# Gustavroot/DeflatedMLMC_Schwinger

Measured on AMD Instinct MI355X. Metric: hutchinson_probe_samples_per_sec_schwinger128, higher is better.
Workload: dtype f64

## Files before the change

### deflatedmlmc_schwinger_amd/csrc/sw_engine.hip

```cpp
#include "../../include/schwinger_hip.h"
#include "sw_kernels.hpp"
#include "sw_pack.hpp"
#include "sw_poly.hpp"

#include <dlfcn.h>

#include <algorithm>
#include <chrono>
#include <cmath>
#include <complex>
#include <cstdarg>
#include <cstdio>
#include <cstdlib>
#include <cstring>
#include <functional>
#include <map>
#include <mutex>
#include <string>
#include <type_traits>
#include <vector>

using swk::cplx;
using swk::cplxf;
using swk::PtrList;
// ... 66 lines not shown
  cplx* h2 = nullptr;
  cplx* c1 = nullptr;
  cplx* nrm = nullptr;
  cplx* gram = nullptr;
};

struct Level {
  int n = 0;
  bool stencil = false;
  int L = 0;
  double mass = 0.0;
  cplx* U1 = nullptr;
  cplx* U2 = nullptr;
  EllOp A, P, R;
  EllOp Re;
  EllOp dinv;
  int nu_pre = 0, nu_post = 3, kcycle = 0;
  std::vector<std::complex<double>> w_pre, w_post;
  bool rich = false;
  std::vector<std::complex<double>> w_eo;
  std::vector<std::complex<double>> q_w;
  std::complex<double> q_beta;
  EllOp eo_op[5];
  std::vector<int> h_rowmap;
  int* rowmap = nullptr;
  int ws_nbp = 0;
  cplx *b = nullptr, *x = nullptr, *r = nullptr, *t = nullptr;
  cplxf *U1f = nullptr, *U2f = nullptr;
  int ws32_nbp = 0;
  cplxf *b32 = nullptr, *x32 = nullptr, *r32 = nullptr, *t32 = nullptr, *i32 = nullptr, *o32 = nullptr;
  int gm_m = 0, gm_cycles = 0;
  cplx *g1 = nullptr, *g2 = nullptr;
  KrylovWS gws;
  cplx *tv = nullptr, *tv2 = nullptr;
  KrylovWS kws;
  KrylovWS sws;
};

struct Hier {
  int nlevels = 0;
  Level lv[SW_MAX_LEVELS];
  EllOp cinv;
  bool ready = false;
  bool f32_valid = false;
  bool even_valid = false;
};
// ... 33 lines not shown
  int mfma_small_tiles = 2;
  int sync_hint[SW_MAX_HIER][SW_MAX_LEVELS] = {{0}};
  bool lazy_sync = true;
  int eo_skew = -1;
  bool eo_skew_chunk = false;
  bool gram_cycle = true;
  bool eo_product = true;
  int gj_block = 32;
  int eo_tile = 0;
  int dense_lds = 4;
  int eo_tile_dbg = 0;
  int num_cus = 256;
  bool direct_small = true;
  bool lgmres_aug = true;
  bool stencil_nt = false;
  int stencil_tile = 0;
  int stencil_spw = 0;
  bool cgs2 = false;
  bool verify = true;
  bool inner_cgs2 = false;
  bool pyth_last = true;
  bool eo_solve = true;
  bool eo_direct = true;
  bool precond_f32 = false;
  int kd = 0;
  cplx* U = nullptr;
  int defl_gemm = 0;
  int lkd[SW_MAX_LEVELS] = {0};
  cplx* lV[SW_MAX_LEVELS] = {nullptr};
  int* perm_src[SW_MAX_LEVELS] = {nullptr};
  EllOp rhsmap[SW_MAX_LEVELS];
  cplx* partial = nullptr;
  size_t partial_bytes = 0;
  cplx* small = nullptr;
  size_t small_bytes = 0;
  void* stage = nullptr;
  size_t stage_bytes = 0;
  std::vector<std::pair<void*, size_t>> allocs;
  int pb_level = -1, pb_nb = 0, pb_nbp = 0;
  int8_t* pb_probes = nullptr;
  struct ProbeSlot {
    int8_t* p = nullptr;
    size_t bytes = 0;
    int level = -1, nb = 0;
    hipEvent_t ready = nullptr;
    bool pending = false;
// ... 100 lines not shown
                                "gj_block must be 0 or a multiple of 8 in 8..256"),
    field<&sw_engine::stencil_nt>("stencil_nt"),
    field<&sw_engine::stencil_tile>("stencil_tile"),
    field<&sw_engine::stencil_spw>("stencil_spw",
                                   [](double v) {
                                     const int t = (int)v;
                                     return t == 0 || t == 1 || t == 2 || t == 4 || t == 8;
                                   },
                                   "stencil_spw must be 0,1,2,4,8"),
    field<&sw_engine::eo_tile>("eo_tile", [](double v) { return v == 0.0 || v == 4.0 || v == 8.0; },
                               "eo_tile must be 0 (off), 4 or 8 waves"),
    {"eo_tile_dbg", get_field<&sw_engine::eo_tile_dbg>, [](sw_engine* h, double v) { h->eo_tile_dbg = (int)v & 3; }},
    field<&sw_engine::eo_skew>("eo_skew", [](double v) { return !(v < -1.0 || v > 65536.0); },
                               "eo_skew must be -1 (automatic), 0 (off) or a strip height"),
    field<&sw_engine::eo_skew_chunk>("eo_skew_chunk"),
    field<&sw_engine::eo_product>("eo_product"),
    field<&sw_engine::p_even>("p_even"),
    {"ell_order", get_field<&sw_engine::ell_order>, [](sw_engine* h, double v) {
       h->ell_order = v != 0.0;
       for (Hier& H : h->hier) H.even_valid = false;
     }},
    field<&sw_engine::direct_small>("direct_small"),
    field<&sw_engine::eo_direct>("eo_direct"),
    field<&sw_engine::lgmres_aug>("lgmres_aug"),
    field<&sw_engine::cgs2>("cgs2"),
    field<&sw_engine::inner_cgs2>("inner_cgs2"),
    field<&sw_engine::pyth_last>("pyth_last"),
    field<&sw_engine::verify>("verify"),
    field<&sw_engine::lazy_sync>("lazy_sync"),
    field<&sw_engine::eo_solve>("eo_solve"),
    field<&sw_engine::gram_cycle>("gram_cycle"),
    field<&sw_engine::stop_factor>("stop_factor", [](double v) { return v > 0.0 && v <= 1.0; },
                                   "stop_factor must be in (0, 1]"),
    field<&sw_engine::precond_f32>("precond_f32"),
    field<&sw_engine::f32_krylov>("f32_krylov"),
    field<&sw_engine::f32_pairs>("f32_pairs"),
    field<&sw_engine::f32_tiles>("f32_tiles",
                                 [](double v) { const int t = (int)v; return t == 0 || t == 1 || t == 2 || t == 4; },
                                 "f32_tiles must be 0, 1, 2 or 4"),
    field<&sw_engine::f32_stages>("f32_stages"),
    field<&sw_engine::f32_dense_stages>("f32_dense_stages"),
    field<&sw_engine::f32_splitk>("f32_splitk"),
    field<&sw_engine::bench_what>("bench_what", [](double v) { return !(v < 0.0 || v > 3.0); },
                                  "bench_what must be 0..3"),
    field<&sw_engine::bench_mode>("bench_mode", [](double v) { return v == 0.0 || v == 1.0 || v == 2.0; },
                                  "bench_mode must be 0, 1 or 2"),
// ... 287 lines not shown
  for (int rt = 0; rt < RT; ++rt) {
    const int ot = tmap ? tmap[rt] : rt;
    for (int r = 0; r < 4; ++r)
      if (kcol[(size_t)rt * KS + KS - 4 + r] != 16 * ot + 4 * r) return;
  }
  op.bsr_diag_last = true;
}

static int free_op(sw_engine* h, EllOp& op) {
  SWCHK(dev_free(h, op.cols));
  SWCHK(dev_free(h, op.vals));
  SWCHK(dev_free(h, op.order));
  SWCHK(dev_free(h, op.order_even));
  SWCHK(dev_free(h, op.bsr_kcol));
  SWCHK(dev_free(h, op.bsr_vals));
  SWCHK(dev_free(h, op.bsr_tmap));
  SWCHK(dev_free(h, op.vals32));
  SWCHK(dev_free(h, op.bsr_vals32));
  op = EllOp();
  return 0;
}

static int launch_bsr(sw_engine* h, const EllOp& op, int mode, const cplx* X, const cplx* B, cplx* Y,
                      int nbp, int cat, cplx w) {
  const int RT = op.bsr_RT > 0 ? op.bsr_RT : op.nrows / 16;
  int NT = h->mfma_tiles;
  if (h->mfma_small_tiles > 0 && (long long)RT * ((2 * nbp) / (16 * NT)) < 4096)
    NT = h->mfma_small_tiles;
  const int bmap = (cat == T_COARSEST) ? h->dense_map : h->bsr_map, msub = h->bsr_sub;
  const int RBn = (RT + SW_WAVES_PER_BLOCK - 1) / SW_WAVES_PER_BLOCK, NCn = (2 * nbp) / (16 * NT);
  const int want = (cat == T_COARSEST) ? h->dense_stages : h->bsr_stages;
  const int stages = (want >= 8 && op.bsr_KS % 8 == 0) ? 8 : ((want >= 4 && op.bsr_KS % 4 == 0) ? 4 : 2);
  dim3 grid = (bmap == 0) ? dim3(RBn, NCn) : dim3(RBn * NCn);
  const int n1 = h->hier[h->solver_hid].nlevels > 1 ? h->hier[h->solver_hid].lv[1].n : 0;
  const int cls = cat == T_COARSEST ? T_MFMA_DENSE
                                    : (cat == T_MVM ? (op.nrows == n1 || n1 == 0 ? T_MFMA_OP : T_MFMA_OP2)
                                                    : cat);
  if (h->profiling) h->twork[cls] += 512.0 * (double)RT * (double)op.bsr_KS * (double)nbp;
  const int dl_kb = 4;
  if (h->mfma_3m && h->dense_lds > 0 && cat == T_COARSEST && mode == 0 && op.dense_uniform &&
      RT % h->dense_lds == 0 && op.bsr_KS % (dl_kb * SW_DL_DEPTH) == 0 && op.bsr_KS >= 2 * dl_kb * SW_DL_DEPTH &&
      (nbp & 31) == 0 && X != Y) {
    return pick<4, 2>(h->dense_lds, [&](auto RTW) {
      return launch(h, cls, swk::k_dense_mfma3_lds<RTW, dl_kb>, dim3((RT / RTW) * (nbp / 32)), dim3(128 * RTW),
                    (const cplx*)op.bsr_vals, (const int*)op.bsr_kcol, op.bsr_KS, RT, X, Y, nbp,
                    (const int*)op.bsr_tmap);
    });
  }
  if (h->mfma_3m) {
    int NT3 = 1;
    if (cat != T_COARSEST && (long long)RT * (nbp / 32) >= 16384) NT3 = 2;
    if (h->mfma3_tiles == 1 || h->mfma3_tiles == 2 || h->mfma3_tiles == 4) NT3 = h->mfma3_tiles;
    while (NT3 > 1 && nbp % (16 * NT3)) NT3 >>= 1;
    const int NC3 = nbp / (16 * NT3);
    const dim3 grid3(RBn * NC3);
    const bool ntio3 = h->bsr_nt && cat != T_COARSEST;
    const int xr = (op.bsr_diag_last && h->bsr_xreg) ? 1 : 0;
    const int bm3 = (bmap == 0) ? 0 : bmap;
    auto b3 = [&](auto MD, auto NTT, auto NTB, auto SG) {
      return launch(h, cls, swk::k_bsr_mfma3<MD, NTT, NTB, SG>, grid3, dim3(SW_BLOCK), (const cplx*)op.bsr_vals,
                    (const int*)op.bsr_kcol, op.bsr_KS, RT, X, B, Y, nbp, w, bm3, msub, (const int*)op.bsr_tmap, xr);
    };
    if (!ntio3 && mode == 0 && want >= 16 && NT3 == 1 && op.bsr_KS % 16 == 0)
      return b3(IntC<0>{}, IntC<1>{}, IntC<0>{}, IntC<16>{});
    if (!ntio3 && mode == 0 && want >= 8)
      return pick<4, 2, 1>(NT3, [&](auto NTT) { return b3(IntC<0>{}, NTT, IntC<0>{}, IntC<8>{}); });
    return pick<0, 1, 3>(mode, [&](auto MD) {
      return pick<4, 2, 1>(NT3, [&](auto NTT) {
        return pick<0, 1>(ntio3, [&](auto NTB) { return b3(MD, NTT, NTB, IntC<4>{}); });
      });
    });
  }
  const bool ntio = h->bsr_nt && cat != T_COARSEST;
  const int xr = (op.bsr_diag_last && h->bsr_xreg) ? 1 : 0;
  return pick<0, 1, 3>(mode, [&](auto MD) {
    return pick<2, 4>(NT, [&](auto NTT) {
      return pick<0, 1>(ntio, [&](auto NTB) {
        return pick<8, 4, 2>(stages, [&](auto SG) {
          return launch(h, cls, swk::k_bsr_mfma<MD, NTT, NTB, SG>, grid, dim3(SW_BLOCK), (const cplx*)op.bsr_vals,
                        (const int*)op.bsr_kcol, op.bsr_KS, RT, (const double*)X, (const double*)B, (double*)Y,
                        2 * nbp, nbp, w, bmap, msub, (const int*)op.bsr_tmap, xr);
        });
      });
    });
  });
// ... 8 lines not shown
  const dim3 grid((ng + SW_WAVES_PER_BLOCK - 1) / SW_WAVES_PER_BLOCK, nbp / 64);
  if (op.G != 1 && op.G != 2 && op.G != 4 && op.G != 8 && op.G != 16)
    return sw_fail(h, "unsupported ELL group size %d", op.G);
  return pick<1, 2, 4, 8, 16>(op.G, [&](auto G) {
    return pick<0, 1, 2, 3>(mode, [&](auto MODE) {
      return launch(h, cat, swk::k_ell<G, MODE, T>, grid, dim3(SW_BLOCK), (const int*)op.cols, vals, op.K, ng, ord,
                    X, B, Y, nbp, w);
    });
  });
}

static int launch_ell(sw_engine* h, const EllOp& op, int mode, const cplx* X, const cplx* B,
                      cplx* Y, int nbp, int cat, cplx w = cplx{0.0, 0.0}, bool even_only = false) {
  if (!op.set) return sw_fail(h, "operator not set");
  if (op.bsr_KS > 0 && (mode == 0 || mode == 1 || mode == 3) && h->use_mfma &&
      (cat == T_COARSEST || h->mfma_ops))
    return launch_bsr(h, op, mode, X, B, Y, nbp, cat, w);
  if (!op.cols || !op.vals)
    return sw_fail(h, "operator exists in MFMA block-row form only (built on the device): it needs "
                      "use_mfma = mfma_ops = 1");
  return launch_ell_groups<cplx>(h, op, op.vals, mode, X, B, Y, nbp, cat, w, even_only);
}

static int launch_bsr(sw_engine* h, const EllOp& op, int mode, const cplx* X, const cplx* B, cplx* Y,
                      int nbp, int cat, cplx w);
static int ensure_level_ws(sw_engine* h, Level& lv, int nbp);

static int apply_coarsest(sw_engine* h, Hier& H, const cplx* X, cplx* Y, int nbp) {
  Level& lc = H.lv[H.nlevels - 1];
  if (h->eo_direct && H.nlevels > 1 && lc.eo_op[4].set && lc.eo_op[1].set && lc.eo_op[2].set &&
      lc.eo_op[3].set && X != Y) {
    SWCHK(ensure_level_ws(h, lc, nbp));
    SWCHK(launch_bsr(h, lc.eo_op[1], 1, X, X, lc.r, nbp, T_MVM, cplx{0.0, 0.0}));
    SWCHK(launch_bsr(h, lc.eo_op[4], 0, lc.r, nullptr, Y, nbp, T_COARSEST, cplx{0.0, 0.0}));
    SWCHK(launch_bsr(h, lc.eo_op[2], 0, X, nullptr, Y, nbp, T_MVM, cplx{0.0, 0.0}));
    return launch_bsr(h, lc.eo_op[3], 1, Y, Y, Y, nbp, T_MVM, cplx{0.0, 0.0});
  }
  if (!H.cinv.set) return sw_fail(h, "coarsest inverse not set");
  return launch_ell(h, H.cinv, 0, X, nullptr, Y, nbp, T_COARSEST);
}

static int stencil_spw(sw_engine* h, int tile_w) {
  int spw = h->stencil_spw > 0 ? h->stencil_spw : 1;
  while (spw > 1 && tile_w % spw) spw >>= 1;
  return spw;
}

template <class C>
static swk::StencilArgsT<C> stencil_args(sw_engine* h, const Level& lv, int nbp, bool eo) {
  using S = typename swk::scalar_of<C>::type;
  swk::StencilArgsT<C> a;
  a.L = lv.L;
  a.Vh = lv.L * lv.L / 2;
  a.diag = (typename swk::real_of<C>::type)(4.0 + lv.mass);
  if constexpr (std::is_same<C, cplx>::value) {
    a.U1 = lv.U1;
    a.U2 = lv.U2;
  } else {
    a.U1 = lv.U1f;
// ... 627 lines not shown
  }
  return 0;
}

static int eo_smooth(sw_engine* h, Level& lv, const cplx* Bin, cplx* start, cplx* other, cplx* Xout,
                     int nbp) {
  cplx* bp = lv.r;
  SWCHK(eo_hop<0>(h, lv, Bin, Bin, bp, nbp));
  cplx* cur = nullptr;
  SWCHK(schur_steps(h, lv, start, other, bp, nbp, &cur));
  SWCHK(eo_hop<1>(h, lv, Bin, cur, cur, nbp));
  if (cur != Xout) return sw_fail(h, "internal: even-odd smoother ended in the wrong buffer");
  return 0;
}

static int vcycle_rich(sw_engine* h, Hier& H, int l, const cplx* Bin, cplx* Xout, int nbp) {
  Level& lv = H.lv[l];
  Level& lc = H.lv[l + 1];
  SWCHK(ensure_level_ws(h, lv, nbp));
  SWCHK(ensure_level_ws(h, lc, nbp));
  SWCHK(ensure_even_orders(h, H));
  if (!lv.P.set || !lv.R.set) return sw_fail(h, "transfer operators of level %d not set", l);
  const size_t npost = lv.w_post.size();
  if (!lv.stencil && lv.eo_op[4].set && lv.eo_op[1].set && lv.eo_op[2].set && lv.eo_op[3].set &&
      lv.w_pre.empty() && h->eo_direct) {
    SWCHK(launch_bsr(h, lv.eo_op[1], 1, Bin, Bin, lv.r, nbp, T_MVM, cplx{0.0, 0.0}));
    SWCHK(launch_bsr(h, lv.eo_op[4], 0, lv.r, nullptr, Xout, nbp, T_COARSEST, cplx{0.0, 0.0}));
    SWCHK(launch_bsr(h, lv.eo_op[2], 0, Bin, nullptr, Xout, nbp, T_MVM, cplx{0.0, 0.0}));
    return launch_bsr(h, lv.eo_op[3], 1, Xout, Xout, Xout, nbp, T_MVM, cplx{0.0, 0.0});
  }
  cplx* xpre = nullptr;
  if (!lv.w_pre.empty()) {
    SWCHK(rich_steps(h, lv, Bin, Xout, lv.t, lv.w_pre, true, nbp, &xpre));
    SWCHK(apply_op(h, lv, 1, xpre, Bin, lv.r, nbp));
    SWCHK(launch_ell(h, lv.R, 0, lv.r, nullptr, lc.b, nbp, T_R));
  } else {
    SWCHK(launch_ell(h, lv.R, 0, Bin, nullptr, lc.b, nbp, T_R));
  }
  SWCHK(coarse_correction(h, H, l, nbp));
  if (!lv.stencil && !lv.w_eo.empty() && !xpre && lv.eo_op[0].set) {
    const bool odd_steps = (lv.w_eo.size() & 1) != 0;
    cplx* cur = odd_steps ? lv.t : Xout;
    cplx* nxt = odd_steps ? Xout : lv.t;
    SWCHK(launch_ell(h, lv.P, 0, lc.x, nullptr, cur, nbp, T_P, cplx{0.0, 0.0}, true));
    SWCHK(launch_bsr(h, lv.eo_op[1], 1, Bin, Bin, lv.r, nbp, T_MVM, cplx{0.0, 0.0}));
    for (size_t k = 0; k < lv.w_eo.size(); ++k) {
      SWCHK(launch_bsr(h, lv.eo_op[0], 3, cur, lv.r, nxt, nbp, T_MVM,
                       cplx{lv.w_eo[k].real(), lv.w_eo[k].imag()}));
      std::swap(cur, nxt);
    }
    SWCHK(launch_bsr(h, lv.eo_op[2], 0, Bin, nullptr, Xout, nbp, T_MVM, cplx{0.0, 0.0}));
    return launch_bsr(h, lv.eo_op[3], 1, Xout, Xout, Xout, nbp, T_MVM, cplx{0.0, 0.0});
// ... 619 lines not shown
  if (h->h_notconv) (void)hipHostFree(h->h_notconv);
  if (h->stream) (void)hipStreamDestroy(h->stream);
  if (h->gen_stream) (void)hipStreamDestroy(h->gen_stream);
  delete h;
  return 0;
}

int sw_hier_begin(sw_engine* h, int hid, int nlevels) {
  if (!h) return 1;
  if (hid < 0 || hid >= SW_MAX_HIER) return sw_fail(h, "hierarchy id %d out of range", hid);
  if (nlevels < 1 || nlevels > SW_MAX_LEVELS) return sw_fail(h, "nlevels %d out of range", nlevels);
  HIPCHK(hipSetDevice(h->device));
  Hier& H = h->hier[hid];
  for (int l = 0; l < SW_MAX_LEVELS; ++l) h->sync_hint[hid][l] = 0;
  for (int l = 0; l < SW_MAX_LEVELS; ++l) {
    Level& lv = H.lv[l];
    SWCHK(dev_free(h, lv.U1)); SWCHK(dev_free(h, lv.U2));
    SWCHK(free_op(h, lv.A));
    SWCHK(free_op(h, lv.P));
    SWCHK(free_op(h, lv.R));
    SWCHK(free_op(h, lv.Re));
    SWCHK(free_op(h, lv.dinv));
    for (int q = 0; q < 5; ++q) SWCHK(free_op(h, lv.eo_op[q]));
    SWCHK(dev_free(h, lv.rowmap));
    SWCHK(dev_free(h, lv.b)); SWCHK(dev_free(h, lv.x)); SWCHK(dev_free(h, lv.r));
    SWCHK(dev_free(h, lv.t));
    SWCHK(dev_free(h, lv.U1f)); SWCHK(dev_free(h, lv.U2f));
    SWCHK(dev_free(h, lv.b32)); SWCHK(dev_free(h, lv.x32)); SWCHK(dev_free(h, lv.r32));
    SWCHK(dev_free(h, lv.t32)); SWCHK(dev_free(h, lv.i32)); SWCHK(dev_free(h, lv.o32));
    SWCHK(free_krylov(h, lv.kws));
    SWCHK(free_krylov(h, lv.sws));
    SWCHK(free_krylov(h, lv.gws));
    SWCHK(dev_free(h, lv.g1)); SWCHK(dev_free(h, lv.g2));
    SWCHK(dev_free(h, lv.tv)); SWCHK(dev_free(h, lv.tv2));
    lv = Level();
  }
  SWCHK(free_op(h, H.cinv));
  H.nlevels = nlevels;
  H.ready = false;
  H.f32_valid = H.even_valid = false;
  if (hid == 0) {
    h->kd = 0;
    SWCHK(dev_free(h, h->U));
    h->U = nullptr;
    for (int l = 0; l < SW_MAX_LEVELS; ++l) {
      h->lkd[l] = 0;
// ... 452 lines not shown
  SWCHK(op_to_dense(h, lv.A, n, D, nullptr));
  SWCHK(gj_invert(h, D, n));
  SWCHK(dense_to_bsr(h, H.cinv, n, D, n, nullptr, nullptr));
  return stream_sync(h);
}

int sw_get_coarsest_inv(sw_engine* h, int hid, double* dense) {
  SWCHK(check_hier(h, hid, 0, false));
  if (!dense) return sw_fail(h, "bad arguments");
  HIPCHK(hipSetDevice(h->device));
  const EllOp& op = h->hier[hid].cinv;
  if (!op.set) return sw_fail(h, "coarsest inverse missing");
  const int n = op.nrows;
  DevBuf<cplx> D(h);
  SWCHK(dev_realloc(h, &D.p, (size_t)n * n));
  SWCHK(op_to_dense(h, op, n, D, nullptr));
  HIPCHK(hipMemcpyAsync(dense, D, (size_t)n * n * sizeof(cplx), hipMemcpyDeviceToHost, h->stream));
  return stream_sync(h);
}

static int schur_apply(sw_engine* h, Level& lv, int mode, const cplx* X, const cplx* Bp, cplx* Y, int nbp);
static int dot_into(sw_engine* h, const cplx* A, const cplx* Bv, int n, int nbp, cplx* out);

int sw_setup_direct_level(sw_engine* h, int hid, int level) {
  SWCHK(check_hier(h, hid, level, false));
  HIPCHK(hipSetDevice(h->device));
  Hier& H = h->hier[hid];
  H.f32_valid = false;
  Level& lv = H.lv[level];
  const EllOp& S = lv.eo_op[0];
  if (lv.stencil || !S.set || !S.bsr_tmap || S.bsr_RT <= 0 || !lv.eo_op[1].set || !lv.eo_op[2].set ||
      !lv.eo_op[3].set)
    return sw_fail(h, "level %d has no even-odd operators (sw_setup_eo_operators / sw_set_eo_operator)", level);
  const int ne = S.bsr_RT, n = ne * 16, ns = lv.n / 16;
  if (n > 8192) return sw_fail(h, "Schur complement of %d rows too large for the in-engine dense inverse", n);
  std::vector<int> E(ne), erank(ns, -1);
  HIPCHK(hipMemcpy(E.data(), S.bsr_tmap, (size_t)ne * sizeof(int), hipMemcpyDeviceToHost));
  for (int r = 0; r < ne; ++r) {
    if (E[r] < 0 || E[r] >= ns || erank[E[r]] >= 0) return sw_fail(h, "level %d: bad tile map of the Schur operator", level);
    erank[E[r]] = r;
  }
  std::vector<int> kc((size_t)ne * S.bsr_KS);
  HIPCHK(hipMemcpy(kc.data(), S.bsr_kcol, kc.size() * sizeof(int), hipMemcpyDeviceToHost));
  for (int c : kc)
    if (erank[c >> 4] < 0) return sw_fail(h, "level %d: the Schur operator reaches an odd site", level);
  DevBuf<int> d_rank(h), d_E(h);
  SWCHK(upload(h, &d_rank.p, erank.data(), erank.size()));
  SWCHK(upload(h, &d_E.p, E.data(), E.size()));
  DevBuf<cplx> D(h);
  SWCHK(dev_realloc(h, &D.p, (size_t)n * n));
  SWCHK(op_to_dense(h, S, n, D, d_rank));
  SWCHK(gj_invert(h, D, n));
  SWCHK(dense_to_bsr(h, lv.eo_op[4], lv.n, D, n, &E, d_E));
  return stream_sync(h);
}

int sw_setup_level_inverse(sw_engine* h, int hid, int level) {
  SWCHK(check_hier(h, hid, level, false));
  HIPCHK(hipSetDevice(h->device));
  Hier& H = h->hier[hid];
  Level& lv = H.lv[level];
  const int n = lv.n;
  if (lv.stencil) return sw_fail(h, "level %d is the lattice level", level);
  if (n <= 0 || n % 16 || n > 8192) return sw_fail(h, "level %d: size %d not a multiple of 16 or above 8192", level, n);
  if (!lv.A.set) return sw_fail(h, "level %d has no operator", level);
  DevBuf<cplx> D(h);
  SWCHK(dev_realloc(h, &D.p, (size_t)n * n));
  SWCHK(op_to_dense(h, lv.A, n, D, nullptr));
  SWCHK(gj_invert(h, D, n));
  SWCHK(dense_to_bsr(h, lv.dinv, n, D, n, nullptr, nullptr));
  H.f32_valid = false;
  return stream_sync(h);
}

int sw_setup_arnoldi(sw_engine* h, int hid, int level, int which, int degree, uint64_t seed, double* Hout) {
  SWCHK(check_hier(h, hid, level, false));
// ... 111 lines not shown
  if (RT <= 0 || KS <= 0 || (KS & 3) || !tmap || !kcol || !vals) return sw_fail(h, "bad arguments");
  const int tiles = lv.n / 16;
  for (int i = 0; i < RT; ++i)
    if (tmap[i] < 0 || tmap[i] >= tiles) return sw_fail(h, "tile map entry out of range");
  for (size_t i = 0; i < (size_t)RT * KS; ++i)
    if (kcol[i] < 0 || kcol[i] + 4 > lv.n) return sw_fail(h, "k-step column out of range");
  EllOp& op = lv.eo_op[which];
  SWCHK(free_op(h, op));
  if (which < 4) SWCHK(free_op(h, lv.eo_op[4]));
  op.nrows = op.ncols = lv.n;
  op.bsr_RT = RT;
  op.bsr_KS = KS;
  SWCHK(upload(h, &op.bsr_tmap, (const int*)tmap, (size_t)RT));
  SWCHK(upload(h, &op.bsr_kcol, (const int*)kcol, (size_t)RT * KS));
  SWCHK(upload(h, (std::complex<double>**)&op.bsr_vals, (const std::complex<double>*)vals,
               (size_t)RT * KS * 64));
  op.set = true;
  check_diag_last(op, kcol, tmap);
  if (which == 4) {
    bool uni = true;
    for (int r = 1; r < RT && uni; ++r) uni = std::memcmp(kcol, kcol + (size_t)r * KS, sizeof(int32_t) * KS) == 0;
    op.dense_uniform = uni;
  }
  return 0;
}

int sw_setup_eo_operators(sw_engine* h, int hid, int level, int Lc) {
  SWCHK(check_hier(h, hid, level, false));
  HIPCHK(hipSetDevice(h->device));
  Hier& H = h->hier[hid];
  H.f32_valid = H.even_valid = false;
  Level& lv = H.lv[level];
  const int ns = Lc * Lc;
  if (lv.stencil || Lc < 8 || (Lc & 1) || lv.n != ns * 16)
    return sw_fail(h, "level %d is not a block level of %d x %d sites (extent even, >= 8)", level, Lc, Lc);
  const EllOp& A = lv.A;
  if (!A.set || A.bsr_KS != 20 || !A.bsr_vals || !A.bsr_kcol || A.bsr_tmap)
    return sw_fail(h, "level %d has no 5-point block-row operator (20 k-steps per site)", level);
  std::vector<int> kc((size_t)ns * 20);
  HIPCHK(hipMemcpy(kc.data(), A.bsr_kcol, kc.size() * sizeof(int), hipMemcpyDeviceToHost));
  std::vector<int> nbr((size_t)ns * 5);
  auto parity = [&](int s) { return ((s % Lc) + (s / Lc)) & 1; };
  for (int s = 0; s < ns; ++s)
    for (int j = 0; j < 5; ++j) {
      const int t = kc[(size_t)s * 20 + 4 * j] / 16;
      for (int g = 0; g < 4; ++g)
// ... 30 lines not shown
      if (site_at(e, disp[q][0], disp[q][1]) == t) return q;
    return -1;
  };
  struct Built {
    std::vector<int> tmap, kcol;
    int KS;
  };
  auto shape = [&](const std::vector<int>& rows, int nblk, auto&& target) {
    Built b;
    b.KS = 4 * nblk;
    b.tmap = rows;
    b.kcol.resize(rows.size() * (size_t)b.KS);
    for (size_t r = 0; r < rows.size(); ++r)
      for (int q = 0; q < nblk; ++q)
        for (int g = 0; g < 4; ++g) b.kcol[r * b.KS + 4 * q + g] = 16 * target((int)r, q) + 4 * g;
    return b;
  };
  Built bS = shape(E, 9, [&](int r, int q) { return site_at(E[r], disp[q][0], disp[q][1]); });
  Built bF = shape(E, 4, [&](int r, int q) { return nbr[(size_t)E[r] * 5 + q]; });
  Built bG = shape(O, 1, [&](int r, int) { return O[r]; });
  Built bH = shape(O, 4, [&](int r, int q) { return nbr[(size_t)O[r] * 5 + q]; });
  Built* built[4] = {&bS, &bF, &bG, &bH};
  SWCHK(free_op(h, lv.eo_op[4]));
  for (int w = 0; w < 4; ++w) {
    EllOp& op = lv.eo_op[w];
    SWCHK(free_op(h, op));
    op.nrows = op.ncols = lv.n;
    op.bsr_RT = (int)built[w]->tmap.size();
    op.bsr_KS = built[w]->KS;
    SWCHK(upload(h, &op.bsr_tmap, built[w]->tmap.data(), built[w]->tmap.size()));
    SWCHK(upload(h, &op.bsr_kcol, built[w]->kcol.data(), built[w]->kcol.size()));
    SWCHK(dev_realloc(h, &op.bsr_vals, (size_t)op.bsr_RT * op.bsr_KS * 64));
    op.set = true;
    check_diag_last(op, built[w]->kcol.data(), built[w]->tmap.data());
  }
  const cplx* Av = A.bsr_vals;
  auto ablk = [](int s, int j) { return ((long long)s * 20 + 4 * j) * 64; };
  auto oblk = [](int r, int nblk, int q) { return ((long long)r * nblk + q) * 256; };
  DevBuf<int> info(h);
  SWCHK(dev_realloc(h, &info.p, (size_t)1));
  HIPCHK(hipMemsetAsync(info, 0, sizeof(int), h->stream));
  {
    std::vector<long long> so(no), dof(no);
    for (int r = 0; r < no; ++r) {
      so[r] = ablk(O[r], 4);
      dof[r] = oblk(r, 1, 0);
// ... 64 lines not shown
        }
      }
      for (int q = 0; q < 9; ++q) {
        ptr.push_back((int)ao.size());
        for (auto& pr : lists[q]) {
          ao.push_back(pr.first);
          bo.push_back(pr.second);
        }
        io.push_back(q == 8 ? ablk(E[r], 4) : -1);
        oo.push_back(oblk(r, 9, q));
      }
    }
    ptr.push_back((int)ao.size());
    SWCHK(products(ptr, ao, bo, lv.eo_op[1].bsr_vals, Av, io, -1.0, lv.eo_op[0].bsr_vals, oo));
  }
  int hinfo = 0;
  HIPCHK(hipMemcpy(&hinfo, info, sizeof(int), hipMemcpyDeviceToHost));
  if (hinfo != 0) return sw_fail(h, "level %d: a diagonal block of an odd site is singular", level);
  return 0;
}

int sw_apply_eo_operator(sw_engine* h, int hid, int level, int which, int nb, const double* X, double* Y) {
  SWCHK(check_hier(h, hid, level, false));
  if (which < 0 || which > 4 || nb <= 0 || !X || !Y) return sw_fail(h, "sw_apply_eo_operator: bad arguments");
  HIPCHK(hipSetDevice(h->device));
  Level& lv = h->hier[hid].lv[level];
  if (lv.stencil || !lv.eo_op[which].set) return sw_fail(h, "level %d has no even-odd operator %d", level, which);
  const int nbp = pad64(nb);
  cplx *a, *b;
  SWCHK(io_vectors(h, lv, nbp, &a, &b));
  SWCHK(pack_host(h, lv, nb, X, a, nbp));
  SWCHK(zero_vec(h, b, lv.n, nbp));
  SWCHK(launch_bsr(h, lv.eo_op[which], 0, a, nullptr, b, nbp, T_MVM, cplx{0.0, 0.0}));
  return unpack_host(h, lv, nb, b, Y, nbp);
}

int sw_get_level_bsr(sw_engine* h, int hid, int level, int* KS, int32_t* kcol, double* vals) {
  SWCHK(check_hier(h, hid, level, false));
  HIPCHK(hipSetDevice(h->device));
  Level& lv = h->hier[hid].lv[level];
  const EllOp& A = lv.A;
  if (!A.set || A.bsr_KS <= 0) return sw_fail(h, "level %d has no block-row operator", level);
  if (KS) *KS = A.bsr_KS;
  if (!kcol || !vals) return 0;
  SWCHK(stream_sync(h));
  const size_t items = (size_t)(lv.n / 16) * A.bsr_KS;
  HIPCHK(hipMemcpy(kcol, A.bsr_kcol, items * sizeof(int), hipMemcpyDeviceToHost));
  HIPCHK(hipMemcpy(vals, A.bsr_vals, items * 64 * sizeof(cplx), hipMemcpyDeviceToHost));
  return 0;
// ... 1298 lines not shown
```

### deflatedmlmc_schwinger_amd/csrc/sw_kernels.hpp

```cpp
#pragma once
#include <hip/hip_runtime.h>
#include <stdint.h>

namespace swk {

typedef double2 cplx;

#define SW_WAVE 64
#define SW_BLOCK 256
#define SW_WAVES_PER_BLOCK 4

__device__ __forceinline__ cplx cmake(double a, double b) { cplx r; r.x = a; r.y = b; return r; }
__device__ __forceinline__ cplx cadd(cplx a, cplx b) { return cmake(a.x + b.x, a.y + b.y); }
__device__ __forceinline__ cplx csub(cplx a, cplx b) { return cmake(a.x - b.x, a.y - b.y); }
__device__ __forceinline__ cplx cmul(cplx a, cplx b) {
  return cmake(fma(a.x, b.x, -a.y * b.y), fma(a.x, b.y, a.y * b.x));
}
__device__ __forceinline__ cplx cmulc(cplx a, cplx b) {
  return cmake(fma(a.x, b.x, a.y * b.y), fma(a.x, b.y, -a.y * b.x));
}
__device__ __forceinline__ void cfma(cplx& acc, cplx a, cplx b) {
  acc.x = fma(a.x, b.x, acc.x);
  acc.x = fma(-a.y, b.y, acc.x);
  acc.y = fma(a.x, b.y, acc.y);
// ... 715 lines not shown
  }
  cplx mm[STG];
  double xx[STG][NT];
#pragma unroll
  for (int s = 0; s < STG; ++s) SW_BSR_LOAD(mm[s], xx[s], s);
  for (int ks = 0; ks < KS; ks += STG) {
#pragma unroll
    for (int s = 0; s < STG; ++s) {
      const int kn = (ks + s + STG < KS) ? ks + s + STG : ks + s;
      __builtin_amdgcn_sched_barrier(0);
      SW_BSR_MFMA(mm[s], xx[s]);
      __builtin_amdgcn_sched_barrier(0);
      SW_BSR_LOAD(mm[s], xx[s], kn);
    }
  }
#undef SW_BSR_LOAD
#undef SW_BSR_MFMA
  if (MODE == 3 && STG == 4 && xreg) bsr_store<MODE, NT, NTIO>(re, im, rt, c0, lane, tmap, Xr, Br, Yr, ld, w, xx);
  else bsr_store<MODE, NT, NTIO>(re, im, rt, c0, lane, tmap, Xr, Br, Yr, ld, w);
}

#define SW_BSR3_MIN_WAVES(NT_, STG_) (((NT_) <= 2 && (STG_) <= 4) ? 2 : 1)

template <int MODE, int NT, bool NTIO = false, int STG = 4>
__global__ __launch_bounds__(SW_BLOCK, SW_BSR3_MIN_WAVES(NT, STG)) void k_bsr_mfma3(
    const cplx* __restrict__ Ap, const int* __restrict__ kcol, int KS, int RT, const cplx* __restrict__ X,
    const cplx* __restrict__ B, cplx* __restrict__ Y, int nbp, cplx w, int map, int msub,
    const int* __restrict__ tmap, int xreg) {
  const int lane = threadIdx.x & 63;
  const int RB = (RT + SW_WAVES_PER_BLOCK - 1) / SW_WAVES_PER_BLOCK;
  const int NC = gridDim.x / RB;
  int bx, cy;
  if (map == 0 || map == 3 || (RB & 7)) {
    cy = blockIdx.x / RB;
    bx = xcd_remap(blockIdx.x - cy * RB, RB);
  } else {
    const int xcd = blockIdx.x & 7, j = blockIdx.x >> 3, RBx = RB >> 3;
    if (map == 1 || (RBx % msub)) {
      cy = j % NC;
      bx = xcd * RBx + j / NC;
    } else {
      const int per = NC * msub;
      const int sidx = j / per, rem = j - sidx * per;
      cy = rem / msub;
      bx = xcd * RBx + sidx * msub + (rem - cy * msub);
    }
  }
  const int rt = __builtin_amdgcn_readfirstlane(bx * SW_WAVES_PER_BLOCK + (threadIdx.x >> 6));
  if (rt >= RT) return;
  const int c0 = cy * (16 * NT);
  const cplx* a = Ap + (size_t)rt * KS * 64 + lane;
  const int* kc = kcol + (size_t)rt * KS;
  const cplx* b = X + (size_t)(lane >> 4) * nbp + c0 + (lane & 15);
  sw_double4 t1[NT], t2[NT], t3[NT];
#pragma unroll
  for (int t = 0; t < NT; ++t) {
    t1[t] = sw_double4{0.0, 0.0, 0.0, 0.0};
    t2[t] = t1[t];
    t3[t] = t1[t];
  }
#define SW_B3_LOAD(M_, X_, KSI)                                 \
  {                                                             \
    M_ = a[(size_t)(KSI) * 64];                                 \
    const cplx* bk_ = b + (size_t)kc[(KSI)] * nbp;              \
    _Pragma("unroll") for (int t = 0; t < NT; ++t) X_[t] = bk_[t * 16]; \
  }
#define SW_B3_MFMA(M_, X_)                                                                  \
  {                                                                                         \
    const double ms_ = M_.x + M_.y;                                                         \
    _Pragma("unroll") for (int t = 0; t < NT; ++t) {                                        \
      t1[t] = __builtin_amdgcn_mfma_f64_16x16x4f64(M_.x, X_[t].x, t1[t], 0, 0, 0);          \
      t2[t] = __builtin_amdgcn_mfma_f64_16x16x4f64(M_.y, X_[t].y, t2[t], 0, 0, 0);          \
      t3[t] = __builtin_amdgcn_mfma_f64_16x16x4f64(ms_, X_[t].x + X_[t].y, t3[t], 0, 0, 0); \
    }                                                                                       \
  }
  cplx mm[STG];
  cplx xx[STG][NT];
#pragma unroll
  for (int s = 0; s < STG; ++s) SW_B3_LOAD(mm[s], xx[s], (s < KS ? s : 0));
  for (int ks = 0; ks < KS; ks += STG) {
#pragma unroll
    for (int s = 0; s < STG; ++s) {
      if (ks + s < KS) {
        const int kn = (ks + s + STG < KS) ? ks + s + STG : ks + s;
        __builtin_amdgcn_sched_barrier(0);
        SW_B3_MFMA(mm[s], xx[s]);
        __builtin_amdgcn_sched_barrier(0);
// ... 1700 lines not shown
                                                           const int* __restrict__ colsite) {
  const int lane = threadIdx.x & 63;
  const int KS = n >> 2;
  const size_t item = (size_t)blockIdx.x * SW_WAVES_PER_BLOCK + (threadIdx.x >> 6);
  if (item >= (size_t)(n >> 4) * KS) return;
  const int rt = (int)(item / KS), ks = (int)(item - (size_t)rt * KS);
  vals[item * 64 + lane] = D[((size_t)rt * 16 + (lane & 15)) * n + 4 * ks + (lane >> 4)];
  if (lane == 0) kcol[item] = colsite ? colsite[ks >> 2] * 16 + 4 * (ks & 3) : 4 * ks;
}

__global__ __launch_bounds__(SW_BLOCK) void k_colscale(cplx* __restrict__ W, const cplx* __restrict__ nrm2,
                                                       int n, int nbp) {
  const int lane = threadIdx.x & 63;
  const size_t col = (size_t)blockIdx.y * 64 + lane;
  const double q = nrm2[col].x;
  const double sc = q > 0.0 ? 1.0 / sqrt(q) : 0.0;
  for (int r = blockIdx.x * SW_WAVES_PER_BLOCK + (threadIdx.x >> 6); r < n; r += gridDim.x * SW_WAVES_PER_BLOCK) {
    const size_t off = (size_t)r * nbp + col;
    const cplx v = W[off];
    W[off] = cmake(sc * v.x, sc * v.y);
  }
}

__global__ __launch_bounds__(SW_BLOCK) void k_copy_tiles(const cplx* __restrict__ X, const int* __restrict__ tmap,
                                                         int RT, int nbp, cplx* __restrict__ Y) {
  const int lane = threadIdx.x & 63;
  const int item = blockIdx.x * SW_WAVES_PER_BLOCK + (threadIdx.x >> 6);
  if (item >= RT * 16) return;
  const size_t row = (size_t)tmap[item >> 4] * 16 + (item & 15);
  for (int c = lane; c < nbp; c += 64) Y[row * nbp + c] = X[row * nbp + c];
}

__global__ __launch_bounds__(SW_BLOCK) void k_fill_random(cplx* __restrict__ V, int n, int nbp,
                                                          int ncols, unsigned long long seed) {
  const int row = blockIdx.x * SW_WAVES_PER_BLOCK + (threadIdx.x >> 6);
  if (row >= n) return;
  const int col = threadIdx.x & 63;
  if (col >= nbp) return;
  unsigned long long z = seed + 0x9e3779b97f4a7c15ull * ((unsigned long long)row * 64ull + col + 1ull);
  z = (z ^ (z >> 30)) * 0xbf58476d1ce4e5b9ull;
  z = (z ^ (z >> 27)) * 0x94d049bb133111ebull;
  z ^= z >> 31;
  const double re = (double)(z & 0xffffffffull) / 2147483648.0 - 1.0;
  const double im = (double)(z >> 32) / 2147483648.0 - 1.0;
  V[(size_t)row * nbp + col] = (col < ncols) ? cmake(re, im) : cmake(0.0, 0.0);
}
// ... 179 lines not shown
```

Baseline: 35650.

## Fuse even-odd direct solve G and H applications into one two-operand BSR kernel

```diff
diff --git a/deflatedmlmc_schwinger_amd/csrc/sw_engine.hip b/deflatedmlmc_schwinger_amd/csrc/sw_engine.hip
--- a/deflatedmlmc_schwinger_amd/csrc/sw_engine.hip
+++ b/deflatedmlmc_schwinger_amd/csrc/sw_engine.hip
@@ -112,6 +112,7 @@
   std::vector<std::complex<double>> q_w;
   std::complex<double> q_beta;
   EllOp eo_op[5];
+  EllOp eo_gh;
   std::vector<int> h_rowmap;
   int* rowmap = nullptr;
   int ws_nbp = 0;
@@ -191,6 +192,7 @@
   bool pyth_last = true;
   bool eo_solve = true;
   bool eo_direct = true;
+  bool direct_fused = true;
   bool precond_f32 = false;
   int kd = 0;
   cplx* U = nullptr;
@@ -337,6 +339,8 @@
      }},
     field<&sw_engine::direct_small>("direct_small"),
     field<&sw_engine::eo_direct>("eo_direct"),
+    field<&sw_engine::direct_fused>("direct_fused", [](double v) { return v == 0.0 || v == 1.0; },
+                                    "direct_fused must be 0 or 1"),
     field<&sw_engine::lgmres_aug>("lgmres_aug"),
     field<&sw_engine::cgs2>("cgs2"),
     field<&sw_engine::inner_cgs2>("inner_cgs2"),
@@ -670,8 +674,10 @@
 }
 
 static int launch_bsr(sw_engine* h, const EllOp& op, int mode, const cplx* X, const cplx* B, cplx* Y,
-                      int nbp, int cat, cplx w) {
+                      int nbp, int cat, cplx w, const cplx* X2 = nullptr, int k2 = 0) {
   const int RT = op.bsr_RT > 0 ? op.bsr_RT : op.nrows / 16;
+  if (X2 && (!h->mfma_3m || mode != 0 || cat == T_COARSEST || k2 <= 0 || k2 > op.bsr_KS))
+    return sw_fail(h, "internal: a second operand base needs the three-product kernel in mode 0");
   int NT = h->mfma_tiles;
   if (h->mfma_small_tiles > 0 && (long long)RT * ((2 * nbp) / (16 * NT)) < 4096)
     NT = h->mfma_small_tiles;
@@ -707,8 +713,17 @@
     const int bm3 = (bmap == 0) ? 0 : bmap;
     auto b3 = [&](auto MD, auto NTT, auto NTB, auto SG) {
       return launch(h, cls, swk::k_bsr_mfma3<MD, NTT, NTB, SG>, grid3, dim3(SW_BLOCK), (const cplx*)op.bsr_vals,
-                    (const int*)op.bsr_kcol, op.bsr_KS, RT, X, B, Y, nbp, w, bm3, msub, (const int*)op.bsr_tmap, xr);
+                    (const int*)op.bsr_kcol, op.bsr_KS, RT, X, B, Y, nbp, w, bm3, msub, (const int*)op.bsr_tmap, xr,
+                    (const cplx*)nullptr, 0);
     };
+    if (X2)
+      return pick<4, 2, 1>(NT3, [&](auto NTT) {
+        return pick<0, 1>(ntio3, [&](auto NTB) {
+          return launch(h, cls, swk::k_bsr_mfma3<0, NTT, NTB, 4, true>, grid3, dim3(SW_BLOCK),
+                        (const cplx*)op.bsr_vals, (const int*)op.bsr_kcol, op.bsr_KS, RT, X, B, Y, nbp, w, bm3, msub,
+                        (const int*)op.bsr_tmap, 0, X2, k2);
+        });
+      });
     if (!ntio3 && mode == 0 && want >= 16 && NT3 == 1 && op.bsr_KS % 16 == 0)
       return b3(IntC<0>{}, IntC<1>{}, IntC<0>{}, IntC<16>{});
     if (!ntio3 && mode == 0 && want >= 8)
@@ -763,19 +778,26 @@
   return launch_ell_groups<cplx>(h, op, op.vals, mode, X, B, Y, nbp, cat, w, even_only);
 }
 
-static int launch_bsr(sw_engine* h, const EllOp& op, int mode, const cplx* X, const cplx* B, cplx* Y,
-                      int nbp, int cat, cplx w);
 static int ensure_level_ws(sw_engine* h, Level& lv, int nbp);
+
+static bool direct_eo_ready(const Level& lv) {
+  return !lv.stencil && lv.eo_op[4].set && lv.eo_op[1].set && lv.eo_op[2].set && lv.eo_op[3].set;
+}
+static int direct_eo_solve(sw_engine* h, Level& lv, const cplx* Bin, cplx* Xout, int nbp) {
+  const cplx z0{0.0, 0.0};
+  SWCHK(launch_bsr(h, lv.eo_op[1], 1, Bin, Bin, lv.r, nbp, T_MVM, z0));
+  SWCHK(launch_bsr(h, lv.eo_op[4], 0, lv.r, nullptr, Xout, nbp, T_COARSEST, z0));
+  if (h->direct_fused && h->mfma_3m && lv.eo_gh.set)
+    return launch_bsr(h, lv.eo_gh, 0, Xout, nullptr, Xout, nbp, T_MVM, z0, Bin, lv.eo_op[2].bsr_KS);
+  SWCHK(launch_bsr(h, lv.eo_op[2], 0, Bin, nullptr, Xout, nbp, T_MVM, z0));
+  return launch_bsr(h, lv.eo_op[3], 1, Xout, Xout, Xout, nbp, T_MVM, z0);
+}
 
 static int apply_coarsest(sw_engine* h, Hier& H, const cplx* X, cplx* Y, int nbp) {
   Level& lc = H.lv[H.nlevels - 1];
-  if (h->eo_direct && H.nlevels > 1 && lc.eo_op[4].set && lc.eo_op[1].set && lc.eo_op[2].set &&
-      lc.eo_op[3].set && X != Y) {
+  if (h->eo_direct && H.nlevels > 1 && direct_eo_ready(lc) && X != Y) {
     SWCHK(ensure_level_ws(h, lc, nbp));
-    SWCHK(launch_bsr(h, lc.eo_op[1], 1, X, X, lc.r, nbp, T_MVM, cplx{0.0, 0.0}));
-    SWCHK(launch_bsr(h, lc.eo_op[4], 0, lc.r, nullptr, Y, nbp, T_COARSEST, cplx{0.0, 0.0}));
-    SWCHK(launch_bsr(h, lc.eo_op[2], 0, X, nullptr, Y, nbp, T_MVM, cplx{0.0, 0.0}));
-    return launch_bsr(h, lc.eo_op[3], 1, Y, Y, Y, nbp, T_MVM, cplx{0.0, 0.0});
+    return direct_eo_solve(h, lc, X, Y, nbp);
   }
   if (!H.cinv.set) return sw_fail(h, "coarsest inverse not set");
   return launch_ell(h, H.cinv, 0, X, nullptr, Y, nbp, T_COARSEST);
@@ -1449,12 +1471,8 @@
   SWCHK(ensure_even_orders(h, H));
   if (!lv.P.set || !lv.R.set) return sw_fail(h, "transfer operators of level %d not set", l);
   const size_t npost = lv.w_post.size();
-  if (!lv.stencil && lv.eo_op[4].set && lv.eo_op[1].set && lv.eo_op[2].set && lv.eo_op[3].set &&
-      lv.w_pre.empty() && h->eo_direct) {
-    SWCHK(launch_bsr(h, lv.eo_op[1], 1, Bin, Bin, lv.r, nbp, T_MVM, cplx{0.0, 0.0}));
-    SWCHK(launch_bsr(h, lv.eo_op[4], 0, lv.r, nullptr, Xout, nbp, T_COARSEST, cplx{0.0, 0.0}));
-    SWCHK(launch_bsr(h, lv.eo_op[2], 0, Bin, nullptr, Xout, nbp, T_MVM, cplx{0.0, 0.0}));
-    return launch_bsr(h, lv.eo_op[3], 1, Xout, Xout, Xout, nbp, T_MVM, cplx{0.0, 0.0});
+  if (direct_eo_ready(lv) && lv.w_pre.empty() && h->eo_direct) {
+    return direct_eo_solve(h, lv, Bin, Xout, nbp);
   }
   cplx* xpre = nullptr;
   if (!lv.w_pre.empty()) {
@@ -2120,6 +2138,7 @@
     SWCHK(free_op(h, lv.Re));
     SWCHK(free_op(h, lv.dinv));
     for (int q = 0; q < 5; ++q) SWCHK(free_op(h, lv.eo_op[q]));
+    SWCHK(free_op(h, lv.eo_gh));
     SWCHK(dev_free(h, lv.rowmap));
     SWCHK(dev_free(h, lv.b)); SWCHK(dev_free(h, lv.x)); SWCHK(dev_free(h, lv.r));
     SWCHK(dev_free(h, lv.t));
@@ -2618,6 +2637,40 @@
 static int schur_apply(sw_engine* h, Level& lv, int mode, const cplx* X, const cplx* Bp, cplx* Y, int nbp);
 static int dot_into(sw_engine* h, const cplx* A, const cplx* Bv, int n, int nbp, cplx* out);
 
+static int build_gh(sw_engine* h, Level& lv) {
+  SWCHK(free_op(h, lv.eo_gh));
+  const EllOp& G = lv.eo_op[2];
+  const EllOp& Hb = lv.eo_op[3];
+  if (lv.stencil || !G.set || !Hb.set || !G.bsr_tmap || !Hb.bsr_tmap || G.bsr_RT <= 0 || G.bsr_RT != Hb.bsr_RT ||
+      G.bsr_KS <= 0 || Hb.bsr_KS <= 0 || ((G.bsr_KS + Hb.bsr_KS) & 3))
+    return 0;
+  const int RT = G.bsr_RT, kg = G.bsr_KS, kh = Hb.bsr_KS, KS = kg + kh;
+  std::vector<int> tg(RT), th(RT), cg((size_t)RT * kg), ch((size_t)RT * kh), kc((size_t)RT * KS);
+  SWCHK(stream_sync(h));
+  HIPCHK(hipMemcpy(tg.data(), G.bsr_tmap, tg.size() * sizeof(int), hipMemcpyDeviceToHost));
+  HIPCHK(hipMemcpy(th.data(), Hb.bsr_tmap, th.size() * sizeof(int), hipMemcpyDeviceToHost));
+  if (tg != th) return 0;
+  HIPCHK(hipMemcpy(cg.data(), G.bsr_kcol, cg.size() * sizeof(int), hipMemcpyDeviceToHost));
+  HIPCHK(hipMemcpy(ch.data(), Hb.bsr_kcol, ch.size() * sizeof(int), hipMemcpyDeviceToHost));
+  for (int r = 0; r < RT; ++r) {
+    std::copy(ch.begin() + (size_t)r * kh, ch.begin() + (size_t)(r + 1) * kh, kc.begin() + (size_t)r * KS);
+    std::copy(cg.begin() + (size_t)r * kg, cg.begin() + (size_t)(r + 1) * kg, kc.begin() + (size_t)r * KS + kh);
+  }
+  EllOp& op = lv.eo_gh;
+  op.nrows = op.ncols = lv.n;
+  op.bsr_RT = RT;
+  op.bsr_KS = KS;
+  SWCHK(upload(h, &op.bsr_tmap, tg.data(), tg.size()));
+  SWCHK(upload(h, &op.bsr_kcol, kc.data(), kc.size()));
+  SWCHK(dev_realloc(h, &op.bsr_vals, (size_t)RT * KS * 64));
+  const size_t items = (size_t)RT * KS * 64;
+  SWCHK(launch(h, T_OTHER, swk::k_gh_values, dim3((unsigned)((items + SW_BLOCK - 1) / SW_BLOCK)), dim3(SW_BLOCK),
+               (const cplx*)Hb.bsr_vals, (const cplx*)G.bsr_vals, RT, kh, kg, op.bsr_vals));
+  op.set = true;
+  check_diag_last(op, kc.data(), tg.data());
+  return stream_sync(h);
+}
+
 int sw_setup_direct_level(sw_engine* h, int hid, int level) {
   SWCHK(check_hier(h, hid, level, false));
   HIPCHK(hipSetDevice(h->device));
@@ -2648,6 +2701,7 @@
   SWCHK(op_to_dense(h, S, n, D, d_rank));
   SWCHK(gj_invert(h, D, n));
   SWCHK(dense_to_bsr(h, lv.eo_op[4], lv.n, D, n, &E, d_E));
+  SWCHK(build_gh(h, lv));
   return stream_sync(h);
 }
 
@@ -2805,6 +2859,8 @@
     for (int r = 1; r < RT && uni; ++r) uni = std::memcmp(kcol, kcol + (size_t)r * KS, sizeof(int32_t) * KS) == 0;
     op.dense_uniform = uni;
   }
+  if (which < 4) SWCHK(free_op(h, lv.eo_gh));
+  else SWCHK(build_gh(h, lv));
   return 0;
 }
 
@@ -2881,6 +2937,7 @@
   Built bH = shape(O, 4, [&](int r, int q) { return nbr[(size_t)O[r] * 5 + q]; });
   Built* built[4] = {&bS, &bF, &bG, &bH};
   SWCHK(free_op(h, lv.eo_op[4]));
+  SWCHK(free_op(h, lv.eo_gh));
   for (int w = 0; w < 4; ++w) {
     EllOp& op = lv.eo_op[w];
     SWCHK(free_op(h, op));
@@ -2991,9 +3048,20 @@
 
 int sw_apply_eo_operator(sw_engine* h, int hid, int level, int which, int nb, const double* X, double* Y) {
   SWCHK(check_hier(h, hid, level, false));
-  if (which < 0 || which > 4 || nb <= 0 || !X || !Y) return sw_fail(h, "sw_apply_eo_operator: bad arguments");
+  if (which < 0 || which > 5 || nb <= 0 || !X || !Y) return sw_fail(h, "sw_apply_eo_operator: bad arguments");
   HIPCHK(hipSetDevice(h->device));
   Level& lv = h->hier[hid].lv[level];
+  if (which == 5) {
+    if (lv.stencil || !lv.eo_gh.set || !h->mfma_3m)
+      return sw_fail(h, "level %d has no combined even-odd operator (or mfma_3m is off)", level);
+    const int nbp = pad64(nb);
+    cplx *a, *b;
+    SWCHK(io_vectors(h, lv, nbp, &a, &b));
+    SWCHK(pack_host(h, lv, nb, X, a, nbp));
+    SWCHK(zero_vec(h, b, lv.n, nbp));
+    SWCHK(launch_bsr(h, lv.eo_gh, 0, a, nullptr, b, nbp, T_MVM, cplx{0.0, 0.0}, a, lv.eo_op[2].bsr_KS));
+    return unpack_host(h, lv, nb, b, Y, nbp);
+  }
   if (lv.stencil || !lv.eo_op[which].set) return sw_fail(h, "level %d has no even-odd operator %d", level, which);
   const int nbp = pad64(nb);
   cplx *a, *b;
diff --git a/deflatedmlmc_schwinger_amd/csrc/sw_kernels.hpp b/deflatedmlmc_schwinger_amd/csrc/sw_kernels.hpp
--- a/deflatedmlmc_schwinger_amd/csrc/sw_kernels.hpp
+++ b/deflatedmlmc_schwinger_amd/csrc/sw_kernels.hpp
@@ -761,11 +761,12 @@
 
 #define SW_BSR3_MIN_WAVES(NT_, STG_) (((NT_) <= 2 && (STG_) <= 4) ? 2 : 1)
 
-template <int MODE, int NT, bool NTIO = false, int STG = 4>
+template <int MODE, int NT, bool NTIO = false, int STG = 4, bool TWO = false>
 __global__ __launch_bounds__(SW_BLOCK, SW_BSR3_MIN_WAVES(NT, STG)) void k_bsr_mfma3(
     const cplx* __restrict__ Ap, const int* __restrict__ kcol, int KS, int RT, const cplx* __restrict__ X,
     const cplx* __restrict__ B, cplx* __restrict__ Y, int nbp, cplx w, int map, int msub,
-    const int* __restrict__ tmap, int xreg) {
+    const int* __restrict__ tmap, int xreg, const cplx* __restrict__ X2, int k2) {
+  static_assert(!TWO || (MODE == 0 && STG == 4), "the second operand base exists for MODE 0, STG 4");
   const int lane = threadIdx.x & 63;
   const int RB = (RT + SW_WAVES_PER_BLOCK - 1) / SW_WAVES_PER_BLOCK;
   const int NC = gridDim.x / RB;
@@ -791,6 +792,8 @@
   const cplx* a = Ap + (size_t)rt * KS * 64 + lane;
   const int* kc = kcol + (size_t)rt * KS;
   const cplx* b = X + (size_t)(lane >> 4) * nbp + c0 + (lane & 15);
+  const cplx* b2 = TWO ? X2 + (size_t)(lane >> 4) * nbp + c0 + (lane & 15) : b;
+  const int ksplit = TWO ? KS - k2 : KS;
   sw_double4 t1[NT], t2[NT], t3[NT];
 #pragma unroll
   for (int t = 0; t < NT; ++t) {
@@ -801,7 +804,7 @@
 #define SW_B3_LOAD(M_, X_, KSI)                                 \
   {                                                             \
     M_ = a[(size_t)(KSI) * 64];                                 \
-    const cplx* bk_ = b + (size_t)kc[(KSI)] * nbp;              \
+    const cplx* bk_ = ((TWO && (KSI) >= ksplit) ? b2 : b) + (size_t)kc[(KSI)] * nbp; \
     _Pragma("unroll") for (int t = 0; t < NT; ++t) X_[t] = bk_[t * 16]; \
   }
 #define SW_B3_MFMA(M_, X_)                                                                  \
@@ -2548,6 +2551,20 @@
   }
 }
 
+__global__ __launch_bounds__(SW_BLOCK) void k_gh_values(const cplx* __restrict__ Hb, const cplx* __restrict__ G,
+                                                        int RT, int kh, int kg, cplx* __restrict__ out) {
+  const size_t per = (size_t)(kh + kg) * 64, nh = (size_t)kh * 64, ng = (size_t)kg * 64;
+  const size_t i = (size_t)blockIdx.x * SW_BLOCK + threadIdx.x;
+  if (i >= (size_t)RT * per) return;
+  const size_t r = i / per, j = i - r * per;
+  if (j < nh) {
+    const cplx v = Hb[r * nh + j];
+    out[i] = cmake(-v.x, -v.y);
+  } else {
+    out[i] = G[r * ng + (j - nh)];
+  }
+}
+
 __global__ __launch_bounds__(SW_BLOCK) void k_copy_tiles(const cplx* __restrict__ X, const int* __restrict__ tmap,
                                                          int RT, int nbp, cplx* __restrict__ Y) {
   const int lane = threadIdx.x & 63;
```

After: 35700, median of 5. About the same (+0.1%).
